# lenke182/flood-uav-video-segmentation

Hardware: AMD Instinct MI355X
Metric: segmentation FPS @713x713 (PSPNet-ResNet50 keyframe + linear interp, frame_delta=5) (higher is better)
Workload: dtype f32

## Files before the change

flood_uav_video_segmentation_amd/csrc/net_ops.hip:

```cpp
#include "interp.h"
#include "kernels.h"
#include "split.h"

#include <type_traits>

namespace fs {

template <int CPT >
__global__ __launch_bounds__(256) void stem_conv_kernel(StemParams p) {
    extern __shared__ __attribute__((aligned(16))) float wlds[];
    const int taps = p.KH * p.KW * 3;
    for (int i = threadIdx.x; i < taps * p.Cout; i += 256) wlds[i] = p.wgt[i];
    __syncthreads();

    const int groups = p.Cout / CPT;
    const int ppb = 256 / groups;
    const int cg = threadIdx.x % groups;
    const int M = p.B * p.Ho * p.Wo;
    const int m = blockIdx.x * ppb + threadIdx.x / groups;
    if (m >= M) return;
    const int hw = p.Ho * p.Wo;
    const int b = m / hw;
    const int rem = m - b * hw;
    const int oy = rem / p.Wo, ox = rem - oy * p.Wo;
// ... 159 lines not shown
#pragma unroll
        for (int e = 0; e < 8; ++e) wv[e] = 16 * st + 8 * hh + e < taps ? wv[e] : 0.f;
        split8(wv, q);
#pragma unroll
        for (int pl = 0; pl < 3; ++pl) wl[((pl * nsteps + st) * 2 + hh) * p.Cout + n] = q[pl];
    }
    stem_tap_table(p, f, taps, kpad, koff, kyx);
    __syncthreads();
    const int lane = threadIdx.x & 63, wave = threadIdx.x >> 6, i = lane & 31, h = lane >> 5;
    const int M = p.B * p.Ho * p.Wo;
    const __amdgpu_buffer_rsrc_t o_rsrc = __builtin_amdgcn_make_buffer_rsrc((void*)p.out, 0, (unsigned)((long long)M * p.ld_out * 4), 0x00020000);
    const int tiles = (M + 31) / 32;
    for (int tile = blockIdx.x * 4 + wave; tile < tiles; tile += gridDim.x * 4) {
        const int m = tile * 32 + i;
        const StemPixel px = stem_pixel(p, f, m < M ? m : 0);
        const int iy0 = px.iy0, ix0 = px.ix0;
        const float* origin = px.origin;
        f32x16 acc[NT];
#pragma unroll
        for (int j = 0; j < NT; ++j)
#pragma unroll
            for (int e = 0; e < 16; ++e) acc[j][e] = 0.f;
        const int centre = p.pad * rowW + p.pad;
        auto gather = [&](int st, float (&av)[8]) -> unsigned {
            const i32x4* ko = reinterpret_cast<const i32x4*>(koff + 16 * st + 8 * h);
            const i32x4* ky = reinterpret_cast<const i32x4*>(kyx + 16 * st + 8 * h);
            const i32x4 o4[2] = {ko[0], ko[1]}, y4[2] = {ky[0], ky[1]};
            unsigned okbits = 0;
#pragma unroll
            for (int e = 0; e < 8; ++e) {
                const int yx = y4[e >> 2][e & 3];
                const int iy = iy0 + (yx >> 16), ix = ix0 + (yx & 0xffff);
                const bool ok = ((unsigned)iy < (unsigned)p.H) & ((unsigned)ix < (unsigned)p.W);
                av[e] = origin[ok ? o4[e >> 2][e & 3] : centre];
                okbits |= (unsigned)ok << e;
            }
            return okbits;
        };
        for (int c0 = 0; c0 < nsteps; c0 += PF) {
            float raw[PF][8];
            unsigned okb[PF];
#pragma unroll
            for (int j = 0; j < PF; ++j) okb[j] = gather(min(c0 + j, nsteps - 1), raw[j]);
#pragma unroll
            for (int j = 0; j < PF; ++j) {
                const int st = c0 + j;
                if (st < nsteps) {
                    u32x4 a3[3];
                    float x[8];
#pragma unroll
                    for (int e = 0; e < 8; ++e) x[e] = (okb[j] >> e) & 1 ? raw[j][e] : 0.f;
                    split8(x, a3);
#pragma unroll
                    for (int term = 0; term < 6; ++term)
#pragma unroll
                        for (int jn = 0; jn < NT; ++jn)
                            acc[jn] = __builtin_amdgcn_mfma_f32_32x32x16_bf16(__builtin_bit_cast(bf16x8, a3[SPLIT_PA[term]]),
                                                                              __builtin_bit_cast(bf16x8, wl[((SPLIT_PB[term] * nsteps + st) * 2 + h) * p.Cout + jn * 32 + i]), acc[jn], 0, 0, 0);
                }
            }
        }
        stem_store_tile(acc, p, o_rsrc, tile, i, h);
    }
#endif
}

int launch_stem_conv(const StemParams& p, hipStream_t s) {
    FS_REQUIRE(p.Cout >= 16 && p.Cout <= 256 && p.Cout % 16 == 0, "stem_conv: unsupported Cout=%d", p.Cout);
    FS_REQUIRE(p.ld_out % 4 == 0, "stem_conv: ld_out must be a multiple of 4");
    FS_REQUIRE((long long)p.B * p.Ho * p.Wo * p.ld_out * 4 < (1ll << 31), "stem_conv: output tensor must be smaller than 2 GiB");
    const FrameSrc& f = p.src;
    if (f.ncrops) {
        FS_REQUIRE(f.ncrops <= 32 && f.in && (p.B == f.ncrops || (p.B == 2 * f.ncrops && f.in2)), "stem_conv: bad crop batch (%d crops, B=%d)", f.ncrops, p.B);
        for (int c = 0; c < f.ncrops; ++c)
            FS_REQUIRE(f.cy[c] >= 0 && f.cx[c] >= 0 && f.cy[c] + p.H <= f.FH && f.cx[c] + p.W <= f.FW, "stem_conv: crop %d (%d,%d)+%dx%d outside the %dx%d frame",
                       c, f.cy[c], f.cx[c], p.H, p.W, f.FH, f.FW);
    } else {
        FS_REQUIRE(f.B1 >= 0 && f.B1 <= p.B && (f.B1 == p.B || f.in2) && (f.B1 == 0 || f.in), "stem_conv: bad frame split B1=%d of B=%d", f.B1, p.B);
    }
    const int M = p.B * p.Ho * p.Wo;
    const int taps = p.KH * p.KW * 3;
    if (p.split && p.Cout % 32 == 0 && p.Cout <= 128 && p.KH < 0x7fff) {
        const int nsteps = cdiv(taps, 16);
        const size_t lds = (size_t)3 * 16 * nsteps * p.Cout * 2 + (size_t)2 * 16 * nsteps * sizeof(int);
        FS_REQUIRE(lds <= 150 * 1024, "stem_conv: filter planes %zu B exceed the LDS budget", lds);
        FS_REQUIRE((long long)3 * (f.ncrops ? (long long)f.FH * f.FW : (long long)p.H * p.W) < (1ll << 31), "stem_conv: frame too large for 32-bit tap offsets");
        const int tiles = cdiv(M, 32);
        const int per_cu = (int)std::max<size_t>(1, std::min<size_t>(8, (size_t)160 * 1024 / lds));
        const dim3 grid((unsigned)std::min(cdiv(tiles, 4), 256 * per_cu));
#define FS_STEM_SPLIT_PF(NT_, PF_)                                                                                               \
    {                                                                                                                            \
        if (lds > 64 * 1024)                                                                                                     \
            FS_HIP(hipFuncSetAttribute(reinterpret_cast<const void*>(&stem_conv_split_kernel<NT_, PF_>), hipFuncAttributeMaxDynamicSharedMemorySize, (int)lds)); \
        hipLaunchKernelGGL((stem_conv_split_kernel<NT_, PF_>), grid, dim3(256), lds, s, p, nsteps);                              \
    }
#define FS_STEM_SPLIT(NT_)                                                                                                       \
    {                                                                                                                            \
        if (nsteps <= 2) FS_STEM_SPLIT_PF(NT_, 2) else FS_STEM_SPLIT_PF(NT_, 5)                                                  \
    }
        switch (p.Cout / 32) {
            case 1: FS_STEM_SPLIT(1) break;
            case 2: FS_STEM_SPLIT(2) break;
            case 3: FS_STEM_SPLIT(3) break;
            default: FS_STEM_SPLIT(4) break;
        }
#undef FS_STEM_SPLIT
#undef FS_STEM_SPLIT_PF
        FS_HIP(hipGetLastError());
        return 0;
    }
    if (p.Cout % 32 == 0 && p.Cout <= 128 && p.KH < 0x7fff) {
        const int ksteps = cdiv(cdiv(taps, 2), 8) * 8;
        const size_t lds = (size_t)2 * ksteps * (p.Cout + 2) * sizeof(float);
        FS_REQUIRE(lds <= 128 * 1024, "stem_conv: filter bank %zu B exceeds LDS budget", lds);
        FS_REQUIRE((long long)3 * (f.ncrops ? (long long)f.FH * f.FW : (long long)p.H * p.W) < (1ll << 31), "stem_conv: frame too large for 32-bit tap offsets");
        const int tiles = cdiv(M, 32);
        const dim3 grid((unsigned)std::min(cdiv(tiles, 4), 256 * 8));
#define FS_STEM_LAUNCH(NT_)                                                                                                      \
    {                                                                                                                            \
        if (lds > 64 * 1024)                                  \
            FS_HIP(hipFuncSetAttribute(reinterpret_cast<const void*>(&stem_conv_mfma_kernel<NT_>), hipFuncAttributeMaxDynamicSharedMemorySize, (int)lds)); \
        hipLaunchKernelGGL((stem_conv_mfma_kernel<NT_>), grid, dim3(256), lds, s, p, ksteps);                                    \
    }
        switch (p.Cout / 32) {
            case 1: FS_STEM_LAUNCH(1) break;
            case 2: FS_STEM_LAUNCH(2) break;
            case 3: FS_STEM_LAUNCH(3) break;
            default: FS_STEM_LAUNCH(4) break;
        }
#undef FS_STEM_LAUNCH
        FS_HIP(hipGetLastError());
        return 0;
    }
    FS_REQUIRE(256 % (p.Cout / 16) == 0, "stem_conv: the VALU kernel needs Cout / 16 to divide 256 (Cout=%d)", p.Cout);
    const int groups = p.Cout / 16, ppb = 256 / groups;
    const size_t lds = (size_t)taps * p.Cout * sizeof(float);
    FS_REQUIRE(lds <= 64 * 1024, "stem_conv: filter bank %zu B exceeds LDS budget", lds);
    hipLaunchKernelGGL((stem_conv_kernel<16>), dim3(cdiv(M, ppb)), dim3(256), lds, s, p);
    FS_HIP(hipGetLastError());
    return 0;
}

__global__ __launch_bounds__(256) void maxpool3x3s2_kernel(const float* __restrict__ in, int ld_in, float* __restrict__ out,
                                                           int ld_out, int B, int H, int W, int C4, int Ho, int Wo) {
    const unsigned r = blockIdx.x * 256 + threadIdx.x;
    if (r >= (unsigned)(Wo * C4)) return;
    const int ox = (int)(r / (unsigned)C4), c4 = (int)(r - (unsigned)ox * (unsigned)C4);
    for (int b = blockIdx.z; b < B; b += gridDim.z) {
        for (int oy = blockIdx.y; oy < Ho; oy += gridDim.y) {
            f32x4 tap[9];
#pragma unroll
            for (int ky = 0; ky < 3; ++ky) {
                const int iy = min(max(oy * 2 - 1 + ky, 0), H - 1);
#pragma unroll
                for (int kx = 0; kx < 3; ++kx) {
                    const int ix = min(max(ox * 2 - 1 + kx, 0), W - 1);
                    tap[ky * 3 + kx] = *reinterpret_cast<const f32x4*>(in + ((size_t)(b * H + iy) * W + ix) * ld_in + c4 * 4);
                }
            }
            f32x4 best = {-INFINITY, -INFINITY, -INFINITY, -INFINITY};
#pragma unroll
            for (int ky = 0; ky < 3; ++ky)
#pragma unroll
                for (int kx = 0; kx < 3; ++kx) {
                    const bool ok = (unsigned)(oy * 2 - 1 + ky) < (unsigned)H && (unsigned)(ox * 2 - 1 + kx) < (unsigned)W;
#pragma unroll
// ... 1 lines not shown
                }
            *reinterpret_cast<f32x4*>(out + ((size_t)(b * Ho + oy) * Wo + ox) * ld_out + c4 * 4) = best;
        }
    }
}

int launch_maxpool3x3s2(const float* in, int ld_in, float* out, int ld_out, int B, int H, int W, int C, int Ho, int Wo,
                        hipStream_t s) {
    FS_REQUIRE(C % 4 == 0 && ld_in % 4 == 0 && ld_out % 4 == 0, "maxpool: C/ld must be multiples of 4");
    FS_REQUIRE((int64_t)Wo * (C / 4) < (int64_t)1 << 31, "maxpool: output row too large");
    hipLaunchKernelGGL(maxpool3x3s2_kernel, dim3((unsigned)cdiv(Wo * (C / 4), 256), (unsigned)std::min(Ho, 65535), (unsigned)std::min(B, 65535)), dim3(256), 0, s,
                       in, ld_in, out, ld_out, B, H, W, C / 4, Ho, Wo);
    FS_HIP(hipGetLastError());
    return 0;
}

__global__ __launch_bounds__(256) void adaptive_avgpool_kernel(const float* __restrict__ in, int ld_in, float* __restrict__ out,
                                                               int H, int W, int C, int bin) {
    __shared__ f32x4 part[32][8];
    const int cell = blockIdx.x, b = blockIdx.z;
    const int by = cell / bin, bx = cell - by * bin;
    const int ys = (by * H) / bin, ye = ((by + 1) * H + bin - 1) / bin;
    const int xs = (bx * W) / bin, xe = ((bx + 1) * W + bin - 1) / bin;
    const int wh = ye - ys, ww = xe - xs;
    const int cl = threadIdx.x & 7, pg = threadIdx.x >> 3;
    const int c = blockIdx.y * 32 + cl * 4;
    f32x4 acc = {0.f, 0.f, 0.f, 0.f};
    for (int i = pg; i < wh * ww; i += 32) {
        const int y = ys + i / ww, x = xs + i % ww;
        const f32x4 v = *reinterpret_cast<const f32x4*>(in + ((size_t)(b * H + y) * W + x) * ld_in + c);
        acc += v;
    }
    part[pg][cl] = acc;
    __syncthreads();
    if (pg == 0) {
        f32x4 sum = part[0][cl];
        for (int g = 1; g < 32; ++g) sum += part[g][cl];
        const float inv = 1.f / (float)(wh * ww);
        sum *= inv;
        *reinterpret_cast<f32x4*>(out + ((size_t)b * bin * bin + cell) * C + c) = sum;
    }
}

int launch_adaptive_avgpool(const float* in, int ld_in, float* out, int B, int H, int W, int C, int bin, hipStream_t s) {
    FS_REQUIRE(C % 32 == 0 && ld_in % 4 == 0, "adaptive_avgpool: C=%d must be a multiple of 32", C);
    hipLaunchKernelGGL(adaptive_avgpool_kernel, dim3(bin * bin, C / 32, B), dim3(256), 0, s, in, ld_in, out, H, W, C, bin);
    FS_HIP(hipGetLastError());
    return 0;
}

__global__ __launch_bounds__(256) void ppm_pool_combine_kernel(const float* __restrict__ cell_mean , float* __restrict__ out1,
                                                               float* __restrict__ out2, float* __restrict__ out3, int B, int C) {
    const int64_t total = (int64_t)B * C;
    for (int64_t i = (int64_t)blockIdx.x * 256 + threadIdx.x; i < total; i += (int64_t)gridDim.x * 256) {
        const int c = (int)(i % C), b = (int)(i / C);
        const float* m = cell_mean + (size_t)b * 36 * C + c;
        float s3[9], s2[4] = {0.f, 0.f, 0.f, 0.f}, s1 = 0.f;
#pragma unroll
        for (int k = 0; k < 9; ++k) s3[k] = 0.f;
#pragma unroll
        for (int y = 0; y < 6; ++y)
#pragma unroll
            for (int x = 0; x < 6; ++x) {
                const float v = m[(size_t)(y * 6 + x) * C];
                s3[(y / 2) * 3 + x / 2] += v;
                s2[(y / 3) * 2 + x / 3] += v;
                s1 += v;
            }
#pragma unroll
        for (int k = 0; k < 9; ++k) out3[((size_t)b * 9 + k) * C + c] = s3[k] * 0.25f;
#pragma unroll
        for (int k = 0; k < 4; ++k) out2[((size_t)b * 4 + k) * C + c] = s2[k] * (1.f / 9.f);
        out1[(size_t)b * C + c] = s1 * (1.f / 36.f);
    }
}

int launch_ppm_pool_combine(const float* cell_mean, float* out1, float* out2, float* out3, int B, int C, hipStream_t s) {
    const int64_t total = (int64_t)B * C;
    hipLaunchKernelGGL(ppm_pool_combine_kernel, dim3((unsigned)cdiv64(total, 256)), dim3(256), 0, s, cell_mean, out1, out2, out3, B, C);
    FS_HIP(hipGetLastError());
    return 0;
}

template <int KV >
__global__ __launch_bounds__(256) void rowdot_1x1_kernel(RowdotBatch pb, int ld_in, int ld_out, int K, int N, int relu) {
    const RowdotProblem& q = pb.p[blockIdx.z];
    const int lane = threadIdx.x & 63;
    const int n = blockIdx.x * 4 + (threadIdx.x >> 6);
    if (n >= N) return;
    const int M = q.M;
    const int per = (M + gridDim.y - 1) / gridDim.y;
    const int m_begin = blockIdx.y * per, m_end = min(M, (int)(blockIdx.y + 1) * per);
    if (m_begin >= m_end) return;
    f32x4 w[KV];
#pragma unroll
    for (int i = 0; i < KV; ++i) w[i] = *reinterpret_cast<const f32x4*>(q.wgt + (size_t)n * K + (i * 64 + lane) * 4);
    const float sc = q.scale ? q.scale[n] : 1.f, sh = q.shift ? q.shift[n] : 0.f;
    for (int m = m_begin; m < m_end; ++m) {
        float acc = 0.f;
#pragma unroll
        for (int i = 0; i < KV; ++i) {
            const f32x4 x = *reinterpret_cast<const f32x4*>(q.in + (size_t)m * ld_in + (i * 64 + lane) * 4);
            acc += x[0] * w[i][0] + x[1] * w[i][1] + x[2] * w[i][2] + x[3] * w[i][3];
        }
#pragma unroll
        for (int off = 32; off > 0; off >>= 1) acc += __shfl_xor(acc, off, 64);
        if (lane == 0) {
            float y = acc * sc + sh;
            if (relu) y = fmaxf(y, 0.f);
            q.out[(size_t)m * ld_out + n] = y;
        }
    }
}

int launch_rowdot_1x1_batch(const RowdotBatch& pb, int nprob, int ld_in, int ld_out, int K, int N, int relu, hipStream_t s) {
    FS_REQUIRE(K % 256 == 0 && K <= 4096, "rowdot_1x1: K=%d must be a multiple of 256 and <= 4096", K);
    FS_REQUIRE(nprob >= 1 && nprob <= 4, "rowdot_1x1: 1..4 problems per launch");
    int mmax = 1;
    for (int i = 0; i < nprob; ++i) mmax = std::max(mmax, pb.p[i].M);
    const dim3 grid(cdiv(N, 4), std::max(1, std::min(12, mmax / 6)), nprob), block(256);
#define FS_ROWDOT(KV)                                                                                             \
    case KV:                                                                                                      \
        hipLaunchKernelGGL((rowdot_1x1_kernel<KV>), grid, block, 0, s, pb, ld_in, ld_out, K, N, relu);            \
        break;
    switch (K / 256) {
        FS_ROWDOT(1) FS_ROWDOT(2) FS_ROWDOT(3) FS_ROWDOT(4) FS_ROWDOT(5) FS_ROWDOT(6) FS_ROWDOT(7) FS_ROWDOT(8)
        FS_ROWDOT(9) FS_ROWDOT(10) FS_ROWDOT(11) FS_ROWDOT(12) FS_ROWDOT(13) FS_ROWDOT(14) FS_ROWDOT(15) FS_ROWDOT(16)
        default: return fail("rowdot_1x1: unsupported K");
    }
#undef FS_ROWDOT
    FS_HIP(hipGetLastError());
    return 0;
}

int launch_rowdot_1x1(const float* in, int ld_in, const float* wgt, const float* scale, const float* shift, float* out,
                      int ld_out, int M, int K, int N, int relu, hipStream_t s) {
    RowdotBatch pb{};
    pb.p[0] = RowdotProblem{in, wgt, scale, shift, out, M};
    return launch_rowdot_1x1_batch(pb, 1, ld_in, ld_out, K, N, relu, s);
}

int launch_upsample_into(const float* in, int hi, int wi, float* out, int ld_out, int B, int Ho, int Wo, int C,
                         int align_corners, hipStream_t s) {
    FS_REQUIRE(C % 4 == 0 && ld_out % 4 == 0 && ((uintptr_t)out & 15) == 0, "upsample_into: C/ld_out must be multiples of 4");
    return launch_resize_bilinear_nhwc(in, C, B, C, hi, wi, out, ld_out, Ho, Wo, align_corners, s, 256 * 32);
}

__global__ __launch_bounds__(256) void classifier_nchw_kernel(const float* __restrict__ in, int ld_in, const float* __restrict__ wgt,
                                                              const float* __restrict__ bias, float* __restrict__ out, int B,
                                                              int HW, int C, int K) {
    extern __shared__ __attribute__((aligned(16))) float wl[];
    for (int i = threadIdx.x; i < K * C; i += 256) wl[i] = wgt[i];
    __syncthreads();
    const int l16 = threadIdx.x & 15;
    const int64_t M = (int64_t)B * HW;
    const int64_t m = (int64_t)blockIdx.x * 16 + (threadIdx.x >> 4);
    const int64_t mc = m < M ? m : M - 1;
    const float* x = in + (size_t)mc * ld_in;
    for (int k0 = 0; k0 < K; k0 += 8) {
        float acc[8];
#pragma unroll
        for (int k = 0; k < 8; ++k) acc[k] = 0.f;
        for (int c = l16 * 4; c < C; c += 64) {
            const f32x4 v = *reinterpret_cast<const f32x4*>(x + c);
#pragma unroll
            for (int k = 0; k < 8; ++k) {
                if (k0 + k < K) {
                    const f32x4 w = *reinterpret_cast<const f32x4*>(wl + (size_t)(k0 + k) * C + c);
                    acc[k] += v[0] * w[0] + v[1] * w[1] + v[2] * w[2] + v[3] * w[3];
                }
            }
        }
#pragma unroll
        for (int k = 0; k < 8; ++k) {
#pragma unroll
            for (int off = 8; off > 0; off >>= 1) acc[k] += __shfl_xor(acc[k], off, 64);
        }
        if (l16 == 0 && m < M) {
            const int64_t b = m / HW, pix = m - b * HW;
#pragma unroll
            for (int k = 0; k < 8; ++k)
                if (k0 + k < K) out[((size_t)b * K + k0 + k) * HW + pix] = acc[k] + (bias ? bias[k0 + k] : 0.f);
        }
    }
}

int launch_classifier_nchw(const float* in, int ld_in, const float* wgt, const float* bias, float* out, int B, int HW,
                           int C, int K, hipStream_t s) {
    FS_REQUIRE(C % 4 == 0 && ld_in % 4 == 0, "classifier: C must be a multiple of 4");
    const size_t lds = (size_t)K * C * sizeof(float);
    FS_REQUIRE(lds <= 64 * 1024, "classifier: K*C too large for LDS");
    const int64_t M = (int64_t)B * HW;
    hipLaunchKernelGGL(classifier_nchw_kernel, dim3((unsigned)cdiv64(M, 16)), dim3(256), lds, s, in, ld_in, wgt, bias, out, B,
                       HW, C, K);
    FS_HIP(hipGetLastError());
    return 0;
}

__global__ void pack_weights_kernel(const float* __restrict__ w, float* __restrict__ out, int O, int I, int KH, int KW, int hwio) {
    const int64_t total = (int64_t)O * I * KH * KW;
    for (int64_t i = (int64_t)blockIdx.x * blockDim.x + threadIdx.x; i < total; i += (int64_t)gridDim.x * blockDim.x) {
        const int s = (int)(i % KW);
        const int r = (int)((i / KW) % KH);
        const int ci = (int)((i / ((int64_t)KW * KH)) % I);
        const int o = (int)(i / ((int64_t)KW * KH * I));
        size_t dst;
        if (hwio == 1)
            dst = ((size_t)((r * KW + s) * I + ci)) * O + o;
        else if (hwio == 2)
            dst = (((size_t)o * (I / 32) + ci / 32) * KH * KW + r * KW + s) * 32 + (ci & 31);
        else
            dst = ((size_t)((o * KH + r) * KW + s)) * I + ci;
        out[dst] = w[i];
    }
}

int launch_pack_oihw_to_ohwi(const float* w, float* out, int O, int I, int KH, int KW, hipStream_t s) {
    const int64_t total = (int64_t)O * I * KH * KW;
    hipLaunchKernelGGL(pack_weights_kernel, dim3((unsigned)std::min<int64_t>(cdiv64(total, 256), 65535)), dim3(256), 0, s, w, out,
                       O, I, KH, KW, 0);
    FS_HIP(hipGetLastError());
    return 0;
}
int launch_pack_oihw_chunk_major(const float* w, float* out, int O, int I, int KH, int KW, hipStream_t s) {
    FS_REQUIRE(I % 32 == 0, "pack(chunk-major): Cin must be a multiple of 32");
    const int64_t total = (int64_t)O * I * KH * KW;
    hipLaunchKernelGGL(pack_weights_kernel, dim3((unsigned)std::min<int64_t>(cdiv64(total, 256), 65535)), dim3(256), 0, s, w, out,
                       O, I, KH, KW, 2);
    FS_HIP(hipGetLastError());
    return 0;
}
int launch_pack_oihw_to_hwio(const float* w, float* out, int O, int I, int KH, int KW, hipStream_t s) {
    const int64_t total = (int64_t)O * I * KH * KW;
    hipLaunchKernelGGL(pack_weights_kernel, dim3((unsigned)std::min<int64_t>(cdiv64(total, 256), 65535)), dim3(256), 0, s, w, out,
                       O, I, KH, KW, 1);
    FS_HIP(hipGetLastError());
    return 0;
}

__global__ __launch_bounds__(256) void concat_scaled_filters_kernel(const float* __restrict__ wa, const float* __restrict__ sa,
                                                                    const float* __restrict__ ha, int Ka, const float* __restrict__ wb,
                                                                    const float* __restrict__ sb, const float* __restrict__ hb, int Kb,
                                                                    float* __restrict__ out, float* __restrict__ shift_out, int O) {
    const int K = Ka + Kb;
    const int64_t total = (int64_t)O * K;
    for (int64_t i = (int64_t)blockIdx.x * 256 + threadIdx.x; i < total; i += (int64_t)gridDim.x * 256) {
        const int k = (int)(i % K), o = (int)(i / K);
        out[i] = k < Ka ? sa[o] * wa[(size_t)o * Ka + k] : sb[o] * wb[(size_t)o * Kb + (k - Ka)];
        if (k == 0) shift_out[o] = ha[o] + hb[o];
    }
}
int launch_concat_scaled_filters(const float* wa, const float* sa, const float* ha, int Ka, const float* wb, const float* sb, const float* hb,
                                 int Kb, float* out, float* shift_out, int O, hipStream_t s) {
    FS_REQUIRE(wa && sa && ha && wb && sb && hb && out && shift_out && O >= 1 && Ka >= 1 && Kb >= 1, "concat_scaled_filters: bad arguments");
    const int64_t total = (int64_t)O * (Ka + Kb);
    hipLaunchKernelGGL(concat_scaled_filters_kernel, dim3((unsigned)std::min<int64_t>(cdiv64(total, 256), 65535)), dim3(256), 0, s, wa, sa, ha, Ka,
                       wb, sb, hb, Kb, out, shift_out, O);
    FS_HIP(hipGetLastError());
    return 0;
}

__global__ __launch_bounds__(256) void pack_slice_tap_major_kernel(const float* __restrict__ w, float* __restrict__ out, int O, int I,
                                                                   int c0, int nc, int taps) {
    const int64_t total = (int64_t)taps * O * nc;
    for (int64_t i = (int64_t)blockIdx.x * 256 + threadIdx.x; i < total; i += (int64_t)gridDim.x * 256) {
        const int c = (int)(i % nc);
        const int o = (int)((i / nc) % O);
        const int tap = (int)(i / ((int64_t)nc * O));
        out[i] = w[((size_t)o * I + c0 + c) * taps + tap];
    }
}
int launch_pack_slice_tap_major(const float* w, float* out, int O, int I, int c0, int nc, int taps, hipStream_t s) {
    FS_REQUIRE(c0 >= 0 && nc >= 1 && c0 + nc <= I, "pack(slice): channel range outside the filter bank");
    const int64_t total = (int64_t)taps * O * nc;
    hipLaunchKernelGGL(pack_slice_tap_major_kernel, dim3((unsigned)std::min<int64_t>(cdiv64(total, 256), 65535)), dim3(256), 0, s, w, out, O,
                       I, c0, nc, taps);
    FS_HIP(hipGetLastError());
    return 0;
}

constexpr int PPM_P = 6;
constexpr int PPM_J = 12;
struct PpmTermParams {
    float* T; int ld;
    const float* Z[4];
    float* R;
    int bin[4], joff[4];
    float sy[4], sx[4];
    const float* scale; const float* shift;
    int B, H, W, C, relu;
    const float* cls_w; const float* cls_b; float* logits; int K;
};

__global__ __launch_bounds__(256) void ppm_rows_kernel(PpmTermParams p) {
    const int js = blockIdx.x, y = blockIdx.y, b = blockIdx.z;
    const int slot = js / 3, s = js - slot * 3;
    const int c = threadIdx.x * 4;
    if (c >= p.C) return;
    int bi = 3;
    while (slot < p.joff[bi]) --bi;
    const int bin = p.bin[bi], j = slot - p.joff[bi];
    const float* Zb = p.Z[bi] + (size_t)b * bin * bin * 9 * p.C + c;
    f32x4 acc = {0.f, 0.f, 0.f, 0.f};
    for (int r = 0; r < 3; ++r) {
        const int Y = y + r - 1;
        if (Y < 0 || Y >= p.H) continue;
        const LinCoord cy = lin_coord(Y, bin, p.sy[bi], 1);
        const f32x4 z0 = *reinterpret_cast<const f32x4*>(Zb + ((size_t)(cy.i0 * bin + j) * 9 + r * 3 + s) * p.C);
        const f32x4 z1 = *reinterpret_cast<const f32x4*>(Zb + ((size_t)(cy.i1 * bin + j) * 9 + r * 3 + s) * p.C);
#pragma unroll
        for (int e = 0; e < 4; ++e) acc[e] = fmaf(cy.w1, z1[e], fmaf(cy.w0, z0[e], acc[e]));
    }
    *reinterpret_cast<f32x4*>(p.R + (((size_t)(b * p.H + y) * PPM_J + slot) * 3 + s) * p.C + c) = acc;
}

__global__ __launch_bounds__(256) void ppm_term_classify_kernel(PpmTermParams p) {
    const int xt = blockIdx.x, y = blockIdx.y, b = blockIdx.z;
    const int x0 = xt * PPM_P;
    const bool dup = (int)threadIdx.x * 4 >= p.C;
    const int c = dup ? p.C - 4 : (int)threadIdx.x * 4;
    __shared__ int s_j0[4][3], s_nj[4][3];
    __shared__ float wt[4][3][6][PPM_P + 2];
    for (int e = threadIdx.x; e < 4 * 3 * 6 * PPM_P; e += blockDim.x) {
        const int px = e % PPM_P, jj = (e / PPM_P) % 6, s = (e / (6 * PPM_P)) % 3, bi = e / (18 * PPM_P);
        const int pf = max(0, 1 - s - x0), pl = min(PPM_P - 1, min(p.W - 1 - x0, p.W - x0 - s));
        float w = 0.f;
        int j0 = 0, nj = 0;
        if (pf <= pl) {
            const LinCoord cf = lin_coord(x0 + pf + s - 1, p.bin[bi], p.sx[bi], 1), cl = lin_coord(x0 + pl + s - 1, p.bin[bi], p.sx[bi], 1);
            j0 = cf.i0;
            nj = cl.i1 - cf.i0 + 1;
            if (px >= pf && px <= pl) {
                const LinCoord cx = lin_coord(x0 + px + s - 1, p.bin[bi], p.sx[bi], 1);
                const int j = j0 + jj;
                w = (j == cx.i0 ? cx.w0 : 0.f) + (j == cx.i1 ? cx.w1 : 0.f);
            }
        }
        wt[bi][s][jj][px] = w;
        if (px == 0 && jj == 0) {
            s_j0[bi][s] = j0;
            s_nj[bi][s] = nj;
        }
    }
    __syncthreads();
    f32x4 acc[PPM_P];
#pragma unroll
    for (int px = 0; px < PPM_P; ++px) acc[px] = f32x4{0.f, 0.f, 0.f, 0.f};
    const float* Rrow = p.R + (size_t)(b * p.H + y) * PPM_J * 3 * p.C + c;
    for (int bs = 0; bs < 12; ++bs) {
        const int bi = bs / 3, s = bs - bi * 3;
        const int j0 = s_j0[bi][s], nj = s_nj[bi][s];
        for (int jj = 0; jj < nj; ++jj) {
            const f32x4 z = *reinterpret_cast<const f32x4*>(Rrow + ((size_t)(p.joff[bi] + j0 + jj) * 3 + s) * p.C);
#pragma unroll
            for (int px = 0; px < PPM_P; ++px) {
                const float w = wt[bi][s][jj][px];
#pragma unroll
                for (int e = 0; e < 4; ++e) acc[px][e] = fmaf(w, z[e], acc[px][e]);
            }
        }
    }
    const f32x4 sc = p.scale ? *reinterpret_cast<const f32x4*>(p.scale + c) : f32x4{1.f, 1.f, 1.f, 1.f};
    const f32x4 sh = p.shift ? *reinterpret_cast<const f32x4*>(p.shift + c) : f32x4{0.f, 0.f, 0.f, 0.f};
#pragma unroll
    for (int px = 0; px < PPM_P; ++px) {
        const bool in = x0 + px < p.W && !dup;
        const f32x4 v = in ? *reinterpret_cast<const f32x4*>(p.T + ((size_t)(b * p.H + y) * p.W + x0 + px) * p.ld + c) : f32x4{0.f, 0.f, 0.f, 0.f};
#pragma unroll
        for (int e = 0; e < 4; ++e) {
            acc[px][e] = (v[e] + acc[px][e]) * sc[e] + sh[e];
            if (p.relu) acc[px][e] = fmaxf(acc[px][e], 0.f);
            if (dup) acc[px][e] = 0.f;
        }
    }
    constexpr int KC = 8;
    __shared__ float part[PPM_P * KC][16];
    const int nrows = blockDim.x >> 4;
    auto dpp_add = [](float v, auto ctrl) {
        return v + __builtin_bit_cast(float, __builtin_amdgcn_update_dpp(0, __builtin_bit_cast(int, v), decltype(ctrl)::value, 0xf, 0xf, true));
    };
    for (int k0 = 0; k0 < p.K; k0 += KC) {
        const int kc = min(KC, p.K - k0);
        for (int k = 0; k < kc; ++k) {
            const f32x4 w = *reinterpret_cast<const f32x4*>(p.cls_w + (size_t)(k0 + k) * p.C + c);
#pragma unroll
            for (int px = 0; px < PPM_P; ++px) {
                float d = acc[px][0] * w[0] + acc[px][1] * w[1] + acc[px][2] * w[2] + acc[px][3] * w[3];
                d = dpp_add(d, std::integral_constant<int, 0xB1>{});
                d = dpp_add(d, std::integral_constant<int, 0x4E>{});
                d = dpp_add(d, std::integral_constant<int, 0x114>{});
                d = dpp_add(d, std::integral_constant<int, 0x118>{});
                if ((threadIdx.x & 15) == 15) part[px * KC + k][threadIdx.x >> 4] = d;
            }
        }
        __syncthreads();
        if ((int)threadIdx.x < PPM_P * kc) {
            const int px = threadIdx.x / kc, k = threadIdx.x % kc;
            float sum = part[px * KC + k][0];
            for (int r = 1; r < nrows; ++r) sum += part[px * KC + k][r];
            if (x0 + px < p.W) p.logits[(((size_t)b * p.K + k0 + k) * p.H + y) * p.W + x0 + px] = sum + (p.cls_b ? p.cls_b[k0 + k] : 0.f);
        }
        __syncthreads();
    }
}

size_t ppm_term_scratch_floats(int B, int H, int C) { return (size_t)B * H * PPM_J * 3 * C; }

namespace {
int ppm_term_any(float* T, int ld, const float* const Z[4], const int bins[4], float* scratch, const float* scale, const float* shift, int B, int H,
                 int W, int C, int relu, const float* cls_w, const float* cls_b, float* logits, int K, hipStream_t s) {
    FS_REQUIRE(C % 4 == 0 && C <= 1024 && ld % 4 == 0 && ((uintptr_t)T & 15) == 0, "ppm_term_classify: C must be a multiple of 4, <= 1024");
    FS_REQUIRE(logits && cls_w && K >= 1 && ((uintptr_t)cls_w & 15) == 0, "ppm_term_classify: bad classifier");
    FS_REQUIRE(H <= 65535 && B <= 65535, "ppm_term_classify: map too large for the launch grid");
    FS_REQUIRE(bins[0] + bins[1] + bins[2] + bins[3] == PPM_J && scratch, "ppm_term_classify: pyramid levels must add up to %d columns", PPM_J);
    for (int i = 0; i < 4; ++i)
        FS_REQUIRE(bins[i] >= 1 && bins[i] <= 6 && Z[i] && ((uintptr_t)Z[i] & 15) == 0, "ppm_term_classify: bad pyramid level %d (bin %d)", i, bins[i]);
    PpmTermParams p{};
    p.T = T; p.ld = ld; p.R = scratch; p.scale = scale; p.shift = shift;
    p.B = B; p.H = H; p.W = W; p.C = C; p.relu = relu;
    int jo = 0;
    for (int i = 0; i < 4; ++i) {
        p.Z[i] = Z[i];
        p.bin[i] = bins[i];
        p.joff[i] = jo;
        jo += bins[i];
        p.sy[i] = resize_scale(bins[i], H, 1);
        p.sx[i] = resize_scale(bins[i], W, 1);
    }
    p.cls_w = cls_w; p.cls_b = cls_b; p.logits = logits; p.K = K;
    const dim3 block(((C / 4 + 63) / 64) * 64);
    hipLaunchKernelGGL(ppm_rows_kernel, dim3(PPM_J * 3, H, B), block, 0, s, p);
    FS_HIP(hipGetLastError());
    hipLaunchKernelGGL(ppm_term_classify_kernel, dim3(cdiv(W, PPM_P), H, B), block, 0, s, p);
    FS_HIP(hipGetLastError());
    return 0;
}
}

int launch_ppm_term_classify(const float* T, int ld, const float* const Z[4], const int bins[4], float* scratch, const float* scale,
                             const float* shift, int B, int H, int W, int C, int relu, const float* cls_w, const float* cls_b, float* logits_nchw,
                             int K, hipStream_t s) {
    FS_REQUIRE(logits_nchw, "ppm_term_classify: no output");
    return ppm_term_any(const_cast<float*>(T), ld, Z, bins, scratch, scale, shift, B, H, W, C, relu, cls_w, cls_b, logits_nchw, K, s);
}

__global__ __launch_bounds__(256) void nchw_to_nhwc_kernel(const float* __restrict__ in, float* __restrict__ out, int ld_out, int C,
                                                           int HW) {
    __shared__ float tile[32][33];
    const int b = blockIdx.z;
    const int p0 = blockIdx.x * 32, c0 = blockIdx.y * 32;
    const int tx = threadIdx.x & 31, ty = threadIdx.x >> 5;
    for (int r = ty; r < 32; r += 8) {
        const int c = c0 + r, px = p0 + tx;
        tile[r][tx] = (c < C && px < HW) ? in[((size_t)b * C + c) * HW + px] : 0.f;
    }
    __syncthreads();
    for (int r = ty; r < 32; r += 8) {
        const int px = p0 + r, c = c0 + tx;
        if (px < HW && c < C) out[((size_t)b * HW + px) * ld_out + c] = tile[tx][r];
    }
}

__global__ __launch_bounds__(256) void nhwc_to_nchw_kernel(const float* __restrict__ in, int ld_in, float* __restrict__ out, int C,
                                                           int HW) {
    __shared__ float tile[32][33];
    const int b = blockIdx.z;
    const int p0 = blockIdx.x * 32, c0 = blockIdx.y * 32;
    const int tx = threadIdx.x & 31, ty = threadIdx.x >> 5;
    for (int r = ty; r < 32; r += 8) {
        const int px = p0 + r, c = c0 + tx;
        tile[r][tx] = (c < C && px < HW) ? in[((size_t)b * HW + px) * ld_in + c] : 0.f;
    }
    __syncthreads();
    for (int r = ty; r < 32; r += 8) {
        const int c = c0 + r, px = p0 + tx;
        if (px < HW && c < C) out[((size_t)b * C + c) * HW + px] = tile[tx][r];
    }
}

int launch_nchw_to_nhwc(const float* in, float* out, int ld_out, int B, int C, int HW, hipStream_t s) {
// ... 12 lines not shown
```

flood_uav_video_segmentation_amd/csrc/wino_fused.hip:

```cpp
#include "kernels.h"
#include "winograd.h"

namespace fs {

__device__ __forceinline__ int wf_voff(int m, int k) {
    const int g = (0x78 >> ((m >> 1) & 6)) & 3;
    return m * 16 + 4 * ((k >> 2) ^ g) + (k & 3);
}

__device__ __forceinline__ void wf_bt(const float d[6], float t[6]) {
    const float s12 = d[1] + d[2], d12 = d[1] - d[2], s34 = d[3] + d[4], d43 = d[4] - d[3], d42 = d[4] - d[2], d31 = d[3] - d[1];
    t[0] = __builtin_fmaf(4.f, d[0], __builtin_fmaf(-5.f, d[2], d[4]));
    t[1] = __builtin_fmaf(-4.f, s12, s34);
    t[2] = __builtin_fmaf(4.f, d12, d43);
    t[3] = __builtin_fmaf(2.f, d31, d42);
    t[4] = __builtin_fmaf(-2.f, d31, d42);
    t[5] = __builtin_fmaf(4.f, d[1], __builtin_fmaf(-5.f, d[3], d[5]));
}
__device__ __forceinline__ void wf_at(const float m[6], float y[4]) {
    const float s12 = m[1] + m[2], d12 = m[1] - m[2], s34 = m[3] + m[4], d34 = m[3] - m[4];
    y[0] = (m[0] + s12) + s34;
    y[1] = __builtin_fmaf(2.f, d34, d12);
    y[2] = __builtin_fmaf(4.f, s34, s12);
    y[3] = __builtin_fmaf(8.f, d34, d12) + m[5];
// ... 374 lines not shown
    const unsigned u_chunk = (unsigned)p.Cout * 64u;
    const unsigned u_pos = (unsigned)(p.Cin >> 4) * u_chunk;
    const int a_off = wf_voff(m16, 4 * q4);

    f32x4 acc[36];
#pragma unroll
    for (int g = 0; g < 36; ++g) acc[g] = f32x4(0.f);
    f32x4 bq[PD][2];
    auto load_b = [&](int stage, int pair, int slot) {
        const unsigned so = (unsigned)stage * u_chunk + (unsigned)(2 * pair) * u_pos;
        bq[slot][0] = __builtin_bit_cast(f32x4, __builtin_amdgcn_raw_buffer_load_b128(u_rsrc, b_voff, so, 0));
        bq[slot][1] = __builtin_bit_cast(f32x4, __builtin_amdgcn_raw_buffer_load_b128(u_rsrc, b_voff, so + u_pos, 0));
    };
#pragma unroll
    for (int k = 0; k < PD; ++k) load_b(0, k, k);

    int blk = blockIdx.x, ms = 0, ring = 0;
    for (int S = 0; S < total; ++S) {
        __syncthreads();
        const float* vsrc = lds + ring * SUB + a_off;
        const bool more = S + 1 < total;
        const int ns = ms + 1 == nstages ? 0 : ms + 1;
        f32x4 aq[2][2];
        aq[0][0] = *reinterpret_cast<const f32x4*>(vsrc);
        aq[0][1] = *reinterpret_cast<const f32x4*>(vsrc + NT * 16);
#pragma unroll
        for (int k = 0; k < 18; ++k) {
            if (k + 1 < 18) {
                aq[(k + 1) & 1][0] = *reinterpret_cast<const f32x4*>(vsrc + (2 * k + 2) * (NT * 16));
                aq[(k + 1) & 1][1] = *reinterpret_cast<const f32x4*>(vsrc + (2 * k + 3) * (NT * 16));
            }
#pragma unroll
            for (int e = 0; e < 4; ++e) {
                acc[2 * k] = __builtin_amdgcn_mfma_f32_16x16x4f32(aq[k & 1][0][e], bq[k % PD][0][e], acc[2 * k], 0, 0, 0);
                __builtin_amdgcn_sched_barrier(0);
                acc[2 * k + 1] = __builtin_amdgcn_mfma_f32_16x16x4f32(aq[k & 1][1][e], bq[k % PD][1][e], acc[2 * k + 1], 0, 0, 0);
                __builtin_amdgcn_sched_barrier(0);
            }
            if (k + PD < 18) load_b(ms, k + PD, k % PD);
            else if (more) load_b(ns, k + PD - 18, k % PD);
            __builtin_amdgcn_sched_barrier(0);
        }
        if (++ring == NB) ring = 0;
        if (++ms == nstages) {
            wino4_epilogue(acc, p, (blk / ncb) * NT + 4 * q4, n0 + wn * 16 + m16);
#pragma unroll
            for (int g = 0; g < 36; ++g) acc[g] = f32x4(0.f);
            ms = 0;
            blk += G;
        }
    }
#endif
}

size_t wino_fused_bank_floats(int Cin, int Cout) { return (size_t)36 * Cin * Cout; }

bool wino_fused_supported(int Cin, int Cout, int KH, int KW, int stride, int pad, int dil) {
    return KH == 3 && KW == 3 && stride == 1 && pad == 1 && dil == 1 && Cin % 32 == 0 && Cin >= 32 && Cin <= 256 && Cout % 64 == 0;
}

int launch_wino4_fused(const float* in, int ld_in, const float* U, const float* scale, const float* shift, float* out, int ld_out, int B, int H,
                       int W, int Cin, int Cout, int relu, hipStream_t s, int variant) {
    FS_REQUIRE(wino_fused_supported(Cin, Cout, 3, 3, 1, 1, 1), "wino_fused: unsupported shape (Cin=%d Cout=%d)", Cin, Cout);
    FS_REQUIRE(variant == 0 || variant == 2 || variant == 3, "wino_fused: variant %d is not 0, 2 or 3", variant);
    FS_REQUIRE(ld_in >= Cin && ld_out >= Cout && ((uintptr_t)U & 15) == 0 && ((uintptr_t)in & 3) == 0, "wino_fused: bad strides / alignment");
    FS_REQUIRE((int64_t)B * H * W * ld_in * 4 < (int64_t)1 << 30 && (int64_t)B * H * W * ld_out * 4 < (int64_t)1 << 31,
               "wino_fused: input map must be smaller than 1 GiB, output smaller than 2 GiB");
    WinoFusedParams p{};
    p.in = in; p.ld_in = ld_in; p.U = U; p.scale = scale; p.shift = shift; p.out = out; p.ld_out = ld_out;
    p.B = B; p.H = H; p.W = W; p.Cin = Cin; p.Cout = Cout; p.relu = relu;
    p.th = cdiv(H, 4); p.tw = cdiv(W, 4);
    p.T = B * p.th * p.tw;
    const int ncb = Cout / 64;
    if (variant == 0) variant = (int64_t)cdiv(p.T, 16) * ncb > 512 ? 2 : 3;
    if (variant == 3) {
        const int nblk = cdiv(p.T, 16) * ncb;
        hipLaunchKernelGGL((wino4_ws_kernel<6>), dim3(std::min(nblk, 256 - 256 % ncb)), dim3(512), 0, s, p);
    }
    else hipLaunchKernelGGL((wino4_fused_kernel<1, 4>), dim3(cdiv(p.T, 16) * ncb), dim3(256), 0, s, p);
    FS_HIP(hipGetLastError());
    return 0;
}

int launch_wino4_fused_pool(const float* in, int ld_in, const float* U, const float* scale, const float* shift, float* pool, int ld_pool, int B,
                            int H, int W, int Cin, int Cout, hipStream_t s) {
    FS_REQUIRE(wino_fused_supported(Cin, Cout, 3, 3, 1, 1, 1), "wino_fused_pool: unsupported shape (Cin=%d Cout=%d)", Cin, Cout);
    FS_REQUIRE(ld_in >= Cin && ld_pool >= Cout && ((uintptr_t)U & 15) == 0 && ((uintptr_t)in & 3) == 0 && ((uintptr_t)pool & 3) == 0, "wino_fused_pool: bad strides / alignment");
    const int Hp = (H - 1) / 2 + 1, Wp = (W - 1) / 2 + 1;
    FS_REQUIRE((int64_t)B * H * W * ld_in * 4 < (int64_t)1 << 30 && (int64_t)B * Hp * Wp * ld_pool * 4 < (int64_t)1 << 31,
               "wino_fused_pool: input map must be smaller than 1 GiB, pooled map smaller than 2 GiB");
    WinoFusedParams p{};
    p.in = in; p.ld_in = ld_in; p.U = U; p.scale = scale; p.shift = shift; p.out = nullptr; p.ld_out = 0;
    p.B = B; p.H = H; p.W = W; p.Cin = Cin; p.Cout = Cout; p.relu = 1;
    p.th = cdiv(H, 4); p.tw = cdiv(W, 4);
    p.T = B * p.th * p.tw;
    p.pool = pool; p.ld_pool = ld_pool; p.Hp = Hp; p.Wp = Wp; p.nby = cdiv(p.th, 4); p.nbx = cdiv(p.tw, 4);
    FS_HIP(hipMemsetAsync(pool, 0, (size_t)B * Hp * Wp * ld_pool * sizeof(float), s));
    hipLaunchKernelGGL((wino4_fused_kernel<1, 4, true>), dim3((unsigned)(B * p.nby * p.nbx * (Cout / 64))), dim3(256), 0, s, p);
    FS_HIP(hipGetLastError());
    return 0;
}

}
```

Before: 1232.

## Rework rowdot, PPM term classifier and pooled Winograd zeroing

The rowdot 1x1 kernel now stages several input rows in LDS and has each wave walk 4 output channels with prefetched weights, so activations are reused across channels. The grid is flattened over problems by row groups. The PPM term/classify kernel widens its per-thread pixel tile from 6 to 15, builds a compact list of nonzero interpolation rows in LDS, batches Z loads, and preloads classifier weights. The pooled Winograd launch replaces a full memset with a kernel that zeroes only the rim cells, which relies on the fused kernel writing every interior cell. A pad check is also added to the stem split path.

```diff
diff --git a/flood_uav_video_segmentation_amd/csrc/net_ops.hip b/flood_uav_video_segmentation_amd/csrc/net_ops.hip
--- a/flood_uav_video_segmentation_amd/csrc/net_ops.hip
+++ b/flood_uav_video_segmentation_amd/csrc/net_ops.hip
@@ -265,6 +265,8 @@
     const int taps = p.KH * p.KW * 3;
     if (p.split && p.Cout % 32 == 0 && p.Cout <= 128 && p.KH < 0x7fff) {
         const int nsteps = cdiv(taps, 16);
+        FS_REQUIRE(p.KH >= 2 * p.pad + 1 && p.KW >= 2 * p.pad + 1, "stem_conv: a %d x %d window needs pad <= %d on the split route (pad=%d)", p.KH, p.KW,
+                   (std::min(p.KH, p.KW) - 1) / 2, p.pad);
         const size_t lds = (size_t)3 * 16 * nsteps * p.Cout * 2 + (size_t)2 * 16 * nsteps * sizeof(int);
         FS_REQUIRE(lds <= 150 * 1024, "stem_conv: filter planes %zu B exceed the LDS budget", lds);
         FS_REQUIRE((long long)3 * (f.ncrops ? (long long)f.FH * f.FW : (long long)p.H * p.W) < (1ll << 31), "stem_conv: frame too large for 32-bit tap offsets");
@@ -432,46 +434,91 @@
     return 0;
 }
 
+constexpr int ROWDOT_NB = 16;
+struct RowdotGroups { int end[4]; };
+
 template <int KV >
-__global__ __launch_bounds__(256) void rowdot_1x1_kernel(RowdotBatch pb, int ld_in, int ld_out, int K, int N, int relu) {
-    const RowdotProblem& q = pb.p[blockIdx.z];
-    const int lane = threadIdx.x & 63;
-    const int n = blockIdx.x * 4 + (threadIdx.x >> 6);
-    if (n >= N) return;
-    const int M = q.M;
-    const int per = (M + gridDim.y - 1) / gridDim.y;
-    const int m_begin = blockIdx.y * per, m_end = min(M, (int)(blockIdx.y + 1) * per);
-    if (m_begin >= m_end) return;
+__global__ __launch_bounds__(256) void rowdot_1x1_kernel(RowdotBatch pb, RowdotGroups gr, int ld_in, int ld_out, int K, int N, int relu) {
+    constexpr int R = KV <= 8 ? 4 : 2;
+    __shared__ f32x4 xs[R][KV * 64];
+    int pi = 0;
+    while ((int)blockIdx.y >= gr.end[pi]) ++pi;
+    const RowdotProblem& q = pb.p[pi];
+    const int lane = threadIdx.x & 63, wave = threadIdx.x >> 6;
+    const int m0 = ((int)blockIdx.y - (pi ? gr.end[pi - 1] : 0)) * R;
+    const int n0 = blockIdx.x * ROWDOT_NB + wave * (ROWDOT_NB / 4);
     f32x4 w[KV];
-#pragma unroll
-    for (int i = 0; i < KV; ++i) w[i] = *reinterpret_cast<const f32x4*>(q.wgt + (size_t)n * K + (i * 64 + lane) * 4);
-    const float sc = q.scale ? q.scale[n] : 1.f, sh = q.shift ? q.shift[n] : 0.f;
-    for (int m = m_begin; m < m_end; ++m) {
-        float acc = 0.f;
-#pragma unroll
-        for (int i = 0; i < KV; ++i) {
-            const f32x4 x = *reinterpret_cast<const f32x4*>(q.in + (size_t)m * ld_in + (i * 64 + lane) * 4);
-            acc += x[0] * w[i][0] + x[1] * w[i][1] + x[2] * w[i][2] + x[3] * w[i][3];
-        }
-#pragma unroll
-        for (int off = 32; off > 0; off >>= 1) acc += __shfl_xor(acc, off, 64);
+    {
+        const int n = min(n0, N - 1);
+#pragma unroll
+        for (int i = 0; i < KV; ++i) w[i] = *reinterpret_cast<const f32x4*>(q.wgt + (size_t)n * K + (i * 64 + lane) * 4);
+    }
+#pragma unroll
+    for (int r = 0; r < R; ++r) {
+        const float* row = q.in + (size_t)min(m0 + r, q.M - 1) * ld_in;
+#pragma unroll
+        for (int u = 0; u < (KV + 3) / 4; ++u) {
+            const int e = u * 256 + (int)threadIdx.x;
+            if (e < KV * 64) xs[r][e] = *reinterpret_cast<const f32x4*>(row + e * 4);
+        }
+    }
+    __syncthreads();
+#pragma unroll 1
+    for (int j = 0; j < ROWDOT_NB / 4; ++j) {
+        const int n = n0 + j;
+        if (n >= N) break;
+        f32x4 wn[KV];
+        {
+            const int nn = min(n + 1, N - 1);
+#pragma unroll
+            for (int i = 0; i < KV; ++i) wn[i] = *reinterpret_cast<const f32x4*>(q.wgt + (size_t)nn * K + (i * 64 + lane) * 4);
+        }
+        float acc[R];
+#pragma unroll
+        for (int r = 0; r < R; ++r) {
+            acc[r] = 0.f;
+#pragma unroll
+            for (int i = 0; i < KV; ++i) {
+                const f32x4 x = xs[r][i * 64 + lane];
+                acc[r] += x[0] * w[i][0] + x[1] * w[i][1] + x[2] * w[i][2] + x[3] * w[i][3];
+            }
+        }
+#pragma unroll
+        for (int off = 32; off > 0; off >>= 1)
+#pragma unroll
+            for (int r = 0; r < R; ++r) acc[r] += __shfl_xor(acc[r], off, 64);
         if (lane == 0) {
-            float y = acc * sc + sh;
-            if (relu) y = fmaxf(y, 0.f);
-            q.out[(size_t)m * ld_out + n] = y;
-        }
+            const float sc = q.scale ? q.scale[n] : 1.f, sh = q.shift ? q.shift[n] : 0.f;
+#pragma unroll
+            for (int r = 0; r < R; ++r) {
+                float y = acc[r] * sc + sh;
+                if (relu) y = fmaxf(y, 0.f);
+                q.out[(size_t)min(m0 + r, q.M - 1) * ld_out + n] = y;
+            }
+        }
+#pragma unroll
+        for (int i = 0; i < KV; ++i) w[i] = wn[i];
     }
 }
 
 int launch_rowdot_1x1_batch(const RowdotBatch& pb, int nprob, int ld_in, int ld_out, int K, int N, int relu, hipStream_t s) {
     FS_REQUIRE(K % 256 == 0 && K <= 4096, "rowdot_1x1: K=%d must be a multiple of 256 and <= 4096", K);
     FS_REQUIRE(nprob >= 1 && nprob <= 4, "rowdot_1x1: 1..4 problems per launch");
-    int mmax = 1;
-    for (int i = 0; i < nprob; ++i) mmax = std::max(mmax, pb.p[i].M);
-    const dim3 grid(cdiv(N, 4), std::max(1, std::min(12, mmax / 6)), nprob), block(256);
+    const int R = K / 256 <= 8 ? 4 : 2;
+    RowdotGroups gr{};
+    int groups = 0;
+    for (int i = 0; i < 4; ++i) {
+        if (i < nprob) {
+            FS_REQUIRE(pb.p[i].M >= 1, "rowdot_1x1: problem %d has no rows", i);
+            groups += cdiv(pb.p[i].M, R);
+        }
+        gr.end[i] = groups;
+    }
+    FS_REQUIRE(groups <= 65535, "rowdot_1x1: too many rows for the launch grid");
+    const dim3 grid(cdiv(N, ROWDOT_NB), groups), block(256);
 #define FS_ROWDOT(KV)                                                                                             \
     case KV:                                                                                                      \
-        hipLaunchKernelGGL((rowdot_1x1_kernel<KV>), grid, block, 0, s, pb, ld_in, ld_out, K, N, relu);            \
+        hipLaunchKernelGGL((rowdot_1x1_kernel<KV>), grid, block, 0, s, pb, gr, ld_in, ld_out, K, N, relu);        \
         break;
     switch (K / 256) {
         FS_ROWDOT(1) FS_ROWDOT(2) FS_ROWDOT(3) FS_ROWDOT(4) FS_ROWDOT(5) FS_ROWDOT(6) FS_ROWDOT(7) FS_ROWDOT(8)
@@ -629,8 +676,9 @@
     return 0;
 }
 
-constexpr int PPM_P = 6;
+constexpr int PPM_P = 15;
 constexpr int PPM_J = 12;
+constexpr int PPM_ZB = 8;
 struct PpmTermParams {
     float* T; int ld;
     const float* Z[4];
@@ -670,55 +718,77 @@
     const bool dup = (int)threadIdx.x * 4 >= p.C;
     const int c = dup ? p.C - 4 : (int)threadIdx.x * 4;
     __shared__ int s_j0[4][3], s_nj[4][3];
-    __shared__ float wt[4][3][6][PPM_P + 2];
-    for (int e = threadIdx.x; e < 4 * 3 * 6 * PPM_P; e += blockDim.x) {
-        const int px = e % PPM_P, jj = (e / PPM_P) % 6, s = (e / (6 * PPM_P)) % 3, bi = e / (18 * PPM_P);
+    __shared__ float wt[4][3][6][PPM_P + 1];
+    for (int e = threadIdx.x; e < 4 * 3 * PPM_P; e += blockDim.x) {
+        const int px = e % PPM_P, s = (e / PPM_P) % 3, bi = e / (3 * PPM_P);
         const int pf = max(0, 1 - s - x0), pl = min(PPM_P - 1, min(p.W - 1 - x0, p.W - x0 - s));
-        float w = 0.f;
         int j0 = 0, nj = 0;
+        LinCoord cx{-1, -1, 0.f, 0.f};
         if (pf <= pl) {
             const LinCoord cf = lin_coord(x0 + pf + s - 1, p.bin[bi], p.sx[bi], 1), cl = lin_coord(x0 + pl + s - 1, p.bin[bi], p.sx[bi], 1);
             j0 = cf.i0;
             nj = cl.i1 - cf.i0 + 1;
-            if (px >= pf && px <= pl) {
-                const LinCoord cx = lin_coord(x0 + px + s - 1, p.bin[bi], p.sx[bi], 1);
-                const int j = j0 + jj;
-                w = (j == cx.i0 ? cx.w0 : 0.f) + (j == cx.i1 ? cx.w1 : 0.f);
-            }
-        }
-        wt[bi][s][jj][px] = w;
-        if (px == 0 && jj == 0) {
+            if (px >= pf && px <= pl) cx = lin_coord(x0 + px + s - 1, p.bin[bi], p.sx[bi], 1);
+        }
+#pragma unroll
+        for (int jj = 0; jj < 6; ++jj) {
+            const int j = j0 + jj;
+            wt[bi][s][jj][px] = (j == cx.i0 ? cx.w0 : 0.f) + (j == cx.i1 ? cx.w1 : 0.f);
+        }
+        if (px == 0) {
             s_j0[bi][s] = j0;
             s_nj[bi][s] = nj;
         }
     }
     __syncthreads();
+    __shared__ int s_off[72], s_wrow[72], s_ntot;
+    for (int t = threadIdx.x; t < 72; t += blockDim.x) {
+        const int bs = t / 6, jj = t - bs * 6, bi = bs / 3, s = bs - bi * 3;
+        int before = 0;
+        for (int q = 0; q < bs; ++q) before += s_nj[q / 3][q % 3];
+        if (jj < s_nj[bi][s]) {
+            s_off[before + jj] = ((p.joff[bi] + s_j0[bi][s] + jj) * 3 + s) * p.C;
+            s_wrow[before + jj] = t;
+        }
+        if (t == 71) s_ntot = before + s_nj[3][2];
+    }
+    __syncthreads();
+    const int ntot = s_ntot;
     f32x4 acc[PPM_P];
 #pragma unroll
     for (int px = 0; px < PPM_P; ++px) acc[px] = f32x4{0.f, 0.f, 0.f, 0.f};
     const float* Rrow = p.R + (size_t)(b * p.H + y) * PPM_J * 3 * p.C + c;
-    for (int bs = 0; bs < 12; ++bs) {
-        const int bi = bs / 3, s = bs - bi * 3;
-        const int j0 = s_j0[bi][s], nj = s_nj[bi][s];
-        for (int jj = 0; jj < nj; ++jj) {
-            const f32x4 z = *reinterpret_cast<const f32x4*>(Rrow + ((size_t)(p.joff[bi] + j0 + jj) * 3 + s) * p.C);
-#pragma unroll
-            for (int px = 0; px < PPM_P; ++px) {
-                const float w = wt[bi][s][jj][px];
-#pragma unroll
-                for (int e = 0; e < 4; ++e) acc[px][e] = fmaf(w, z[e], acc[px][e]);
+    const float* wrows = &wt[0][0][0][0];
+    for (int t0 = 0; t0 < ntot; t0 += PPM_ZB) {
+        f32x4 z[PPM_ZB];
+#pragma unroll
+        for (int u = 0; u < PPM_ZB; ++u) z[u] = *reinterpret_cast<const f32x4*>(Rrow + s_off[min(t0 + u, ntot - 1)]);
+#pragma unroll
+        for (int u = 0; u < PPM_ZB; ++u) {
+            if (t0 + u < ntot) {
+                const float* wr = wrows + s_wrow[t0 + u] * (PPM_P + 1);
+#pragma unroll
+                for (int px = 0; px < PPM_P; ++px) {
+                    const float w = wr[px];
+#pragma unroll
+                    for (int e = 0; e < 4; ++e) acc[px][e] = fmaf(w, z[u][e], acc[px][e]);
+                }
             }
         }
     }
     const f32x4 sc = p.scale ? *reinterpret_cast<const f32x4*>(p.scale + c) : f32x4{1.f, 1.f, 1.f, 1.f};
     const f32x4 sh = p.shift ? *reinterpret_cast<const f32x4*>(p.shift + c) : f32x4{0.f, 0.f, 0.f, 0.f};
+    f32x4 tv[PPM_P];
 #pragma unroll
     for (int px = 0; px < PPM_P; ++px) {
         const bool in = x0 + px < p.W && !dup;
-        const f32x4 v = in ? *reinterpret_cast<const f32x4*>(p.T + ((size_t)(b * p.H + y) * p.W + x0 + px) * p.ld + c) : f32x4{0.f, 0.f, 0.f, 0.f};
+        tv[px] = in ? *reinterpret_cast<const f32x4*>(p.T + ((size_t)(b * p.H + y) * p.W + x0 + px) * p.ld + c) : f32x4{0.f, 0.f, 0.f, 0.f};
+    }
+#pragma unroll
+    for (int px = 0; px < PPM_P; ++px) {
 #pragma unroll
         for (int e = 0; e < 4; ++e) {
-            acc[px][e] = (v[e] + acc[px][e]) * sc[e] + sh[e];
+            acc[px][e] = (tv[px][e] + acc[px][e]) * sc[e] + sh[e];
             if (p.relu) acc[px][e] = fmaxf(acc[px][e], 0.f);
             if (dup) acc[px][e] = 0.f;
         }
@@ -731,8 +801,13 @@
     };
     for (int k0 = 0; k0 < p.K; k0 += KC) {
         const int kc = min(KC, p.K - k0);
-        for (int k = 0; k < kc; ++k) {
-            const f32x4 w = *reinterpret_cast<const f32x4*>(p.cls_w + (size_t)(k0 + k) * p.C + c);
+        f32x4 cw[KC];
+#pragma unroll
+        for (int k = 0; k < KC; ++k) cw[k] = *reinterpret_cast<const f32x4*>(p.cls_w + (size_t)(k0 + min(k, kc - 1)) * p.C + c);
+#pragma unroll
+        for (int k = 0; k < KC; ++k) {
+            if (k >= kc) break;
+            const f32x4 w = cw[k];
 #pragma unroll
             for (int px = 0; px < PPM_P; ++px) {
                 float d = acc[px][0] * w[0] + acc[px][1] * w[1] + acc[px][2] * w[2] + acc[px][3] * w[3];
@@ -744,8 +819,8 @@
             }
         }
         __syncthreads();
-        if ((int)threadIdx.x < PPM_P * kc) {
-            const int px = threadIdx.x / kc, k = threadIdx.x % kc;
+        for (int t = threadIdx.x; t < PPM_P * kc; t += blockDim.x) {
+            const int px = t / kc, k = t % kc;
             float sum = part[px * KC + k][0];
             for (int r = 1; r < nrows; ++r) sum += part[px * KC + k][r];
             if (x0 + px < p.W) p.logits[(((size_t)b * p.K + k0 + k) * p.H + y) * p.W + x0 + px] = sum + (p.cls_b ? p.cls_b[k0 + k] : 0.f);
diff --git a/flood_uav_video_segmentation_amd/csrc/wino_fused.hip b/flood_uav_video_segmentation_amd/csrc/wino_fused.hip
--- a/flood_uav_video_segmentation_amd/csrc/wino_fused.hip
+++ b/flood_uav_video_segmentation_amd/csrc/wino_fused.hip
@@ -480,6 +480,17 @@
     return 0;
 }
 
+__global__ __launch_bounds__(256) void wino4_pool_zero_rims_kernel(float* __restrict__ pool, int ld_pool, int Hp, int Wp, int Cout) {
+    const int pr = blockIdx.y % Hp;
+    const bool rim_row = (pr & 7) == 0;
+    const int cells = rim_row ? Wp : (Wp + 7) / 8;
+    float* row = pool + (size_t)blockIdx.y * Wp * ld_pool;
+    for (int i = blockIdx.x * 256 + threadIdx.x; i < cells * Cout; i += gridDim.x * 256) {
+        const int cell = i / Cout, ch = i - cell * Cout;
+        row[(size_t)(rim_row ? cell : cell * 8) * ld_pool + ch] = 0.f;
+    }
+}
+
 int launch_wino4_fused_pool(const float* in, int ld_in, const float* U, const float* scale, const float* shift, float* pool, int ld_pool, int B,
                             int H, int W, int Cin, int Cout, hipStream_t s) {
     FS_REQUIRE(wino_fused_supported(Cin, Cout, 3, 3, 1, 1, 1), "wino_fused_pool: unsupported shape (Cin=%d Cout=%d)", Cin, Cout);
@@ -493,7 +504,8 @@
     p.th = cdiv(H, 4); p.tw = cdiv(W, 4);
     p.T = B * p.th * p.tw;
     p.pool = pool; p.ld_pool = ld_pool; p.Hp = Hp; p.Wp = Wp; p.nby = cdiv(p.th, 4); p.nbx = cdiv(p.tw, 4);
-    FS_HIP(hipMemsetAsync(pool, 0, (size_t)B * Hp * Wp * ld_pool * sizeof(float), s));
+    FS_REQUIRE((int64_t)B * Hp <= 65535, "wino_fused_pool: too many pooled rows for the launch grid");
+    hipLaunchKernelGGL(wino4_pool_zero_rims_kernel, dim3((unsigned)cdiv(cdiv(Wp, 8) * Cout, 256), (unsigned)(B * Hp)), dim3(256), 0, s, pool, ld_pool, Hp, Wp, Cout);
     hipLaunchKernelGGL((wino4_fused_kernel<1, 4, true>), dim3((unsigned)(B * p.nby * p.nbx * (Cout / 64))), dim3(256), 0, s, p);
     FS_HIP(hipGetLastError());
     return 0;
```

Result: no change. 1236, median of 4 (+0.3%).
